# akuendig/cuda-matrix-inversion

Measured on AMD Instinct MI355X. Metric: matrix inversions/s, higher is better.
Workload: dtype f64; 1 GPU; gj64: 100000 x 64x64 fp64 Gauss-Jordan, SPD inputs (natural-order pivots verified inside the MFMA sweep; a rejected matrix is redone with partial pivoting), BASELINE configs[2]; n=64, total_batch=100000, batch_per_gpu=100000, algorithm=gj, kernel=matinv_gj_tile_f64<4, true, true>, input=SPD: R + R^T + n I

## Files before the change

cuda-matrix-inversion_amd/_lib.py:

```python
from __future__ import annotations

import ctypes
import os
import subprocess

_HERE = os.path.dirname(os.path.abspath(__file__))
LIB_PATH = os.environ.get("MATINV_LIB", os.path.join(_HERE, "libmatinv_hip.so"))

OK, ERR_ARG, ERR_UNSUPPORTED, ERR_HIP, ERR_NO_DEVICE = 0, -1, -2, -3, -4
F64, F32 = 0, 1
ALGO_GAUSS_JORDAN, ALGO_CHOLESKY = 0, 1
KERNEL_AUTO, KERNEL_LDS, KERNEL_ROWLANE, KERNEL_TILE, KERNEL_ROW, KERNEL_GLOBAL, KERNEL_BLOCKED, KERNEL_TILEP = 0, 1, 2, 3, 4, 5, 6, 7

REFERENCE_GPU_NAMES = [
    "inverse_gauss_batched_gpu", "inverse_lu_cuda_batched_gpu", "inverse_cholesky_stride_batched_gpu",
    "inverse_cholesky_batched_gpu", "inverse_cholesky_mm_batched_gpu", "inverse_cholesky_mm2_batched_gpu",
]
REFERENCE_DEVICE_NAMES = [
    "inverse_gauss_batched_device", "inverse_lu_cuda_batched_device", "inverse_cholesky_stride_batched_device",
    "decompose_cholesky_stride_batched_device", "inverse_upper_stride_batched_device",
    "multiply_upper_stride_batched_device", "inverse_cholesky_batched_device", "decompose_cholesky_batched_device",
    "inverse_cholesky_mm_batched_device", "decompose_cholesky_mm_batched_device",
    "inverse_cholesky_mm2_batched_device",
]
NATIVE_NAMES = [
    "matinv_inverse_batched", "matinv_inverse_batched_ex", "matinv_select_kernel", "matinv_kernel_name",
    "matinv_mean_batched", "matinv_variance_batched", "matinv_inverse_batched_host", "matinv_mean_batched_host",
    "matinv_variance_batched_host", "matinv_last_error",
    "matinv_abi_version", "matinv_release_cache", "matinv_stream_retire", "matinv_batched_malloc", "matinv_batched_free", "matinv_memcpy_2d",
    "matinv_device_synchronize", "matinv_tile_stats", "matinv_queue_create", "matinv_queue_submit", "matinv_queue_submit_chunks", "matinv_queue_pending",
    "matinv_queue_bins", "matinv_queue_flush", "matinv_queue_destroy", "matinv_queue_last_error", "matinv_queue_stream",
    "matinv_set_gj_policy", "matinv_device_count", "matinv_shard_range", "matinv_inverse_batched_host_multi", "matinv_comm_unique_id",
    "matinv_comm_init_rank", "matinv_comm_destroy", "matinv_allgather_shards", "matinv_allgather_local", "matinv_allgather_local_after", "matinv_debug_rejects",
    "matinv_solve_batched", "matinv_solve_batched_ex", "matinv_solve_kernel_name", "matinv_solve_batched_host",
    "matinv_logdet_batched", "matinv_logdet_batched_ex", "matinv_logdet_kernel_name", "matinv_logdet_batched_host",
    "matinv_logml_batched", "matinv_logml_batched_host", "matinv_gp_kernel_name", "matinv_logml_kernel_name",
    "matinv_loo_batched", "matinv_loo_kernel_name", "matinv_loo_batched_host",
    "matinv_logml_grad_batched", "matinv_logml_grad_kernel_name", "matinv_logml_grad_batched_host",
]
GJ_NATURAL_FIRST, GJ_PIVOT, GJ_ADAPTIVE = 0, 1, 2


def build(force: bool = False) -> str:
    if force:
        subprocess.run(["make", "-C", _HERE, "-s", "clean"], check=True)
    subprocess.run(["make", "-C", _HERE, "-s", "-j4"], check=True)
    return LIB_PATH


class MatinvError(RuntimeError):
    def __init__(self, code: int, msg: str):
        super().__init__(f"libmatinv_hip error {code}: {msg}")
        self.code = code
# ... 65 lines not shown
        f.restype = ci
        f.argtypes = [ci, ci, vp, vp, vp, vp, vp, sz, vp]
    L.matinv_inverse_batched_host_multi.restype = ci
    L.matinv_inverse_batched_host_multi.argtypes = [ci, ci, ci, vp, vp, sz, vp, ci]
    L.matinv_set_gj_policy.restype = ci
    L.matinv_set_gj_policy.argtypes = [ci]
    L.matinv_device_count.restype = ci
    L.matinv_shard_range.restype = ci
    L.matinv_shard_range.argtypes = [sz, ci, ci, ci, vp, vp]
    L.matinv_comm_unique_id.restype = ci
    L.matinv_comm_unique_id.argtypes = [vp]
    L.matinv_comm_init_rank.restype = ci
    L.matinv_comm_init_rank.argtypes = [vp, ci, vp, ci]
    L.matinv_comm_destroy.restype = ci
    L.matinv_comm_destroy.argtypes = [vp]
    L.matinv_allgather_shards.restype = ci
    L.matinv_allgather_shards.argtypes = [vp, ci, vp, vp, sz, vp]
    L.matinv_allgather_local.restype = ci
    L.matinv_allgather_local.argtypes = [ci, vp, ci, vp, vp, sz]
    L.matinv_allgather_local_after.restype = ci
    L.matinv_allgather_local_after.argtypes = [ci, vp, ci, vp, vp, sz, vp]
    L.matinv_tile_stats.restype = ci
    L.matinv_tile_stats.argtypes = [vp, vp, vp, vp]
    L.matinv_batched_malloc.restype = ci
    L.matinv_batched_malloc.argtypes = [vp, vp, sz, ci]
    L.matinv_batched_free.restype = ci
    L.matinv_batched_free.argtypes = [vp]
    L.matinv_memcpy_2d.restype = ci
    L.matinv_memcpy_2d.argtypes = [vp, sz, vp, sz, sz, sz, ci]
    L.matinv_device_synchronize.restype = ci
    L.matinv_queue_create.restype = ci
    L.matinv_queue_create.argtypes = [vp, ci, vp, ci]
    L.matinv_queue_submit.restype = ci
    L.matinv_queue_submit.argtypes = [vp, ci, vp, vp, vp, vp, vp, sz, vp]
    L.matinv_queue_submit_chunks.restype = ci
    L.matinv_queue_submit_chunks.argtypes = [vp, sz, vp, vp, vp, vp, vp, vp, vp, vp]
    L.matinv_queue_pending.restype = ci
    L.matinv_queue_pending.argtypes = [vp, vp, vp]
    L.matinv_queue_bins.restype = ci
    L.matinv_queue_bins.argtypes = [vp, vp, ci]
    L.matinv_queue_flush.restype = ci
    L.matinv_queue_flush.argtypes = [vp, vp, vp, vp]
    L.matinv_queue_stream.restype = vp
    L.matinv_queue_stream.argtypes = [vp]
    L.matinv_queue_destroy.restype = ci
    L.matinv_queue_destroy.argtypes = [vp]
# ... 20 lines not shown
```

cuda-matrix-inversion_amd/api.py:

```python
from __future__ import annotations

import ctypes

import numpy as np

from . import _lib
from ._lib import (GJ_ADAPTIVE, GJ_NATURAL_FIRST, GJ_PIVOT,
                   ALGO_CHOLESKY, ALGO_GAUSS_JORDAN, F32, F64, KERNEL_AUTO, KERNEL_BLOCKED, KERNEL_GLOBAL, KERNEL_LDS,
                   KERNEL_ROW, KERNEL_ROWLANE, KERNEL_TILE, KERNEL_TILEP, MatinvError)


def _np_dtype_code(dtype) -> int:
    dtype = np.dtype(dtype)
    if dtype == np.float64:
        return F64
    if dtype == np.float32:
        return F32
    raise TypeError(f"only float32/float64 batches are supported, got {dtype}")


def _torch_dtype_code(t) -> int:
    import torch
    if t.dtype == torch.float64:
        return F64
# ... 404 lines not shown
    return _lib.lib().matinv_logdet_kernel_name(algo, code, n, kernel).decode()


def gp_kernel_name(dtype, n: int, variance: bool = False) -> str:
    code = dtype if isinstance(dtype, int) else _np_dtype_code(dtype)
    return _lib.lib().matinv_gp_kernel_name(code, n, 1 if variance else 0).decode()


def logml_kernel_name(dtype, n: int) -> str:
    code = dtype if isinstance(dtype, int) else _np_dtype_code(dtype)
    return _lib.lib().matinv_logml_kernel_name(code, n).decode()


mean_batched = calcluateMean
variance_batched = calcluateVariance


def tile_stats() -> dict:
    v = [ctypes.c_ulonglong(0) for _ in range(4)]
    _lib.check(_lib.lib().matinv_tile_stats(*[ctypes.byref(x) for x in v]))
    return dict(zip(("natural_launches", "pivot_launches", "last_rejected", "last_batch"), (int(x.value) for x in v)))


def select_kernel(algo: int, dtype, n: int) -> int:
    code = dtype if isinstance(dtype, int) else _np_dtype_code(dtype)
    k = _lib.lib().matinv_select_kernel(algo, code, n)
    if k < 0:
        _lib.check(k)
    return k


def kernel_name(algo: int, dtype, n: int, kernel: int = KERNEL_AUTO) -> str:
    code = dtype if isinstance(dtype, int) else _np_dtype_code(dtype)
    return _lib.lib().matinv_kernel_name(algo, code, n, kernel).decode()
```

cuda-matrix-inversion_amd/csrc/abi.hip:

```cpp
#include <errno.h>
#include <stdarg.h>
#include <stdio.h>
#include <stdlib.h>
#include <string.h>
#include <time.h>

#include <algorithm>
#include <string>
#include <thread>
#include <vector>

#include "../../include/matinv.h"
#include "common.hpp"

using namespace matinv;

namespace {
thread_local char g_err[512] = "";
}

namespace matinv {
int fail(int code, const char *fmt, ...)
{
    va_list ap;
// ... 1016 lines not shown
    return MATINV_OK;
}

int matinv_memcpy_2d(void *dst, size_t dpitch, const void *src, size_t spitch, size_t width, size_t height, int toDevice)
{
    if (width == 0 || height == 0) return MATINV_OK;
    if (!dst || !src || dpitch < width || spitch < width) return fail(MATINV_ERR_ARG, "matinv_memcpy_2d: bad argument");
    hipError_t e = hipMemcpy2D(dst, dpitch, src, spitch, width, height, toDevice ? hipMemcpyHostToDevice : hipMemcpyDeviceToHost);
    if (e != hipSuccess) return fail_hip(e, "hipMemcpy2D");
    return MATINV_OK;
}

int matinv_tile_stats(unsigned long long *natural_launches, unsigned long long *pivot_launches, unsigned long long *last_rejected,
                      unsigned long long *last_batch)
{
    const TileStats s = tile_stats();
    if (natural_launches) *natural_launches = s.natural_launches;
    if (pivot_launches) *pivot_launches = s.pivot_launches;
    if (last_rejected) *last_rejected = s.last_rejected;
    if (last_batch) *last_batch = s.last_batch;
    return MATINV_OK;
}

int matinv_device_synchronize(void)
{
    hipError_t e = hipDeviceSynchronize();
    if (e != hipSuccess) return fail_hip(e, "hipDeviceSynchronize");
    return MATINV_OK;
}

int matinv_inverse_batched_ex(int algo, int dtype, int n, const void *dA, size_t strideA, void *dAinv,
                              size_t strideInv, size_t batch, int *dInfo, void *stream, int kernel)
{
    if (dtype == MATINV_F64)
        return inverse_strided<double>(algo, n, dA, strideA, dAinv, strideInv, batch, dInfo, stream, kernel);
    if (dtype == MATINV_F32)
        return inverse_strided<float>(algo, n, dA, strideA, dAinv, strideInv, batch, dInfo, stream, kernel);
    return fail(MATINV_ERR_ARG, "unknown dtype %d", dtype);
}

int matinv_inverse_batched(int algo, int dtype, int n, const void *dA, size_t strideA, void *dAinv, size_t strideInv,
                           size_t batch, int *dInfo, void *stream)
{
    return matinv_inverse_batched_ex(algo, dtype, n, dA, strideA, dAinv, strideInv, batch, dInfo, stream,
                                     MATINV_KERNEL_AUTO);
}
// ... 277 lines not shown
```

cuda-matrix-inversion_amd/csrc/common.hpp:

```cpp
#pragma once
#include <hip/hip_runtime.h>
#include <stddef.h>
#include <stdint.h>

#include <type_traits>

#include "../../include/matinv.h"

namespace matinv {

typedef unsigned long long hint_t;

int fail(int code, const char *fmt, ...) __attribute__((format(printf, 2, 3)));
int fail_hip(hipError_t e, const char *what);

hipError_t scratch_alloc(void **p, size_t bytes, hipStream_t stream);
hipError_t scratch_free(void *p, hipStream_t stream);
void scratch_retire_stream(hipStream_t stream);
void blocked_gp_release_graphs();
void scratch_release_device();

template <class Body>
hipError_t with_scratch_ints(size_t count, size_t zeroed, hipStream_t stream, Body &&body)
{
// ... 140 lines not shown

template <class T>
hipError_t launch_gj_tile(int n, BatchRef<const T> A, BatchRef<T> X, size_t batch, int *info, hipStream_t stream);
template <class T>
bool tile_family_supports(int n);
bool tile4_supports(int n);
bool tile4_wide_supports(bool f64, int n);
template <class T>
hipError_t launch_gj_tile4(int n, BatchRef<const T> A, BatchRef<T> X, size_t batch, int *info, hipStream_t stream);
template <class T>
hipError_t launch_spd_tile4(int n, BatchRef<const T> A, BatchRef<T> X, size_t batch, int *info, hipStream_t stream);
const char *name_tile4(bool f64, bool spd, int n);
template <class T>
hipError_t launch_spd_tile(int n, BatchRef<const T> A, BatchRef<T> X, size_t batch, int *info, hipStream_t stream);
template <class T>
bool spd_tile_supports(int n);
const char *name_spd_tile(bool f64, int n);

bool tilep_supports(int n);
template <class T>
hipError_t launch_gj_tilep(int n, BatchRef<const T> A, BatchRef<T> X, size_t batch, int *info, hipStream_t stream);
template <class T>
hipError_t launch_gj_tilep_worklist(int n, BatchRef<const T> A, BatchRef<T> X, size_t batch, const int *in_count, const int *in_list,
                                    int *bad_count, int *bad_list, int *info, hipStream_t stream, hint_t *hint_out, bool expect_many = false);
const char *name_gj_tilep(bool f64, int n);
template <class T>
hipError_t launch_gj_tilep4(int n, BatchRef<const T> A, BatchRef<T> X, size_t batch, int *info, hipStream_t stream);
template <class T>
hipError_t launch_gj_tilep4_worklist(int n, BatchRef<const T> A, BatchRef<T> X, size_t batch, const int *in_count, const int *in_list,
                                     int *bad_count, int *bad_list, int *info, hipStream_t stream, hint_t *hint_out, bool expect_many = false);
const char *name_gj_tilep4(bool f64, int n);
template <class T>
hipError_t launch_gj_tileq(int n, BatchRef<const T> A, BatchRef<T> X, size_t batch, int *info, hipStream_t stream, const int *in_count,
                           const int *in_list, hint_t *hint_out, int *bad_count, int *bad_list);
const char *name_gj_tileq(bool f64, int n);
bool tileq_supports(bool f64, int n);
struct TileStats {
    unsigned long long natural_launches, pivot_launches, last_rejected, last_batch;
};
TileStats tile_stats();
bool tile_policy_use_pivot(bool f64, int nt);
hint_t *tile_policy_record(bool f64, int nt, size_t batch);
int gj_policy();
int set_gj_policy(int policy);

const char *name_gj_rowlane(bool f64, int n);
const char *name_gj_tile(bool f64, int n);
template <class T>
hipError_t launch_gp_lds_worklist(int n, const T *As, const T *Bs, const T *Cs, const T *Ds, const T *Es, T *out,
                                  const int *work_count, const int *work_list, int *info, hipStream_t stream);
bool gp_tile_supports(bool f64, int n);
template <class T>
hipError_t launch_gp_tile(int n, const T *As, const T *Bs, const T *Cs, const T *Ds, const T *Es, T *out, size_t batch,
                          int *info, hipStream_t stream);
const char *name_gp_tile(bool f64, int n);
hipError_t debug_note_rejects(const int *work_count, hipStream_t stream);
long long debug_rejects(bool reset);
bool gp_spd_tile_supports(bool f64, int n);
const char *name_gp_spd_tile(bool f64, int n);
int spd_onewave_max(bool f64);
hipError_t enqueue_spd_tile_wide_f32(int n, BatchRef<const float> A, BatchRef<float> X, unsigned grid, unsigned b, int *info, int *ws,
                                     hipStream_t stream);
hipError_t enqueue_spd_tile_wide_f64(int n, BatchRef<const double> A, BatchRef<double> X, unsigned grid, unsigned b, int *info, int *ws,
                                     hipStream_t stream);
// ... 71 lines not shown
```

cuda-matrix-inversion_amd/csrc/tile_impl.hpp:

```cpp
#pragma once
#include <stdio.h>
#include <stdlib.h>
#include <string.h>
#include <atomic>

#include "tile_common.hpp"
#include "tile_screen.hpp"

#ifndef MATINV_TILE_GATED_PANEL
#define MATINV_TILE_GATED_PANEL 1
#endif

#ifndef MATINV_TILE_SYM_SWEEP
#define MATINV_TILE_SYM_SWEEP 1
#endif

namespace matinv {


#define MATINV_PREP_ROW(MOV, b, a) MOV " %" #b ", %" #a "\n\t" MOV " %" #a ", 0\n\t"
#define MATINV_PREP_ZERO(MOV, a) MOV " %" #a ", 0\n\t"
#define MATINV_PREP_TAIL(MOV, save, eye) MOV " %0, %" #eye "\n\ts_nop 1\n\ts_mov_b64 exec, %" #save
#define MATINV_PREP_SAVE(save, mask) "s_and_saveexec_b64 %" #save ", %" #mask "\n\t"
template <int NT, class T>
__device__ __forceinline__ void prep_operands(typename TileGeo<T>::vec4 (&acc)[NT][NT], T (&bop)[NT], int kb, T eye)
{
    static_assert(NT >= 1 && NT <= 4, "prep_operands: one asm text per tile count");
    const int tK = kb >> 2, rK = kb & 3;
    const unsigned long long pmask = sizeof(T) == 8 ? 0x000F000F000F000FULL << (4 * rK) : 0x1111111111111111ULL << rK;
    unsigned long long save;
    auto J = [&](int i) { return (tK + i) % NT; };
    auto R = [&](int i) { return (rK + i) & 3; };
#define ROW(i) acc[tK][J(i)][rK]
#define COL(i, r) acc[J(i)][tK][R(r)]
    if constexpr (sizeof(T) == 8) {
#define MV "v_mov_b64_e32"
        if constexpr (NT == 1)
// ... 387 lines not shown
            if (info && l == 0) info[mat] = 0;                                                                              \
        } else if (l == 0) {                                                                                                \
            const int slot = atomicAdd(work_count, 1);                                                                      \
            work_list[slot] = (int)mat;                                                                                     \
        }
        if constexpr (SYM) {
            auto leave = [&]() {
                MATINV_GJ_TILE_LEAVE
            };
            if (!sym) {
                leave();
            } else {
                int qs = q, cs = c;
                asm volatile("" : "+v"(qs), "+v"(cs));
                wave_lds_sync();
                sym_tile_sweep<NT, MATINV_TILE_GATED_PANEL != 0, T>(acc, panel, qs, cs, bad);
                wave_lds_sync();
                if (bad == 0) sym_tile_finish<NT>(panel, acc, qs, cs);
                leave();
            }
        } else {
            MATINV_GJ_TILE_LEAVE
        }
#undef MATINV_GJ_TILE_LEAVE
        if (LOOKAHEAD) wave_lds_sync();
    }
}


template <int NT, bool FULL, bool LOOKAHEAD, bool EARLY = false>
__global__ __launch_bounds__(64, 2) void matinv_gj_tile_f64(BatchRef<const double> Ain,
                                                                                 BatchRef<double> Xout, int *info,
                                                                                 int n_rt, unsigned batch,
                                                                                 int *work_count, int *work_list, const int *in_count,
                                                                                 const int *in_list)
{
    constexpr bool SYM = MATINV_TILE_SYM_SWEEP && NT == 4 && FULL && LOOKAHEAD;
    __shared__ __attribute__((aligned(16))) double panel[SYM && 16 * NT * 4 < 16 * TILE_TSTRIDE ? 16 * TILE_TSTRIDE : 16 * NT * 4];
    gj_tile_body<double, NT, FULL, LOOKAHEAD, EARLY>(Ain, Xout, info, n_rt, batch, work_count, work_list, panel, in_count, in_list);
}

template <int NT, bool FULL, bool LOOKAHEAD, bool EARLY = false>
__global__ __launch_bounds__(64, FULL ? 4 : 3) void matinv_gj_tile_f32(BatchRef<const float> Ain, BatchRef<float> Xout, int *info,
                                                           int n_rt, unsigned batch, int *work_count, int *work_list, const int *in_count,
                                                           const int *in_list)
{
    __shared__ __attribute__((aligned(16))) float panel[16 * NT * 4];
    gj_tile_body<float, NT, FULL, LOOKAHEAD, EARLY>(Ain, Xout, info, n_rt, batch, work_count, work_list, panel, in_count, in_list);
}

template <class T>
struct SpdGp {
    const T *a, *c, *d, *e;
    T *out;
};

template <class T, int NT, bool FULL, bool GP = false>
__device__ __forceinline__ void spd_tile_body(BatchRef<const T> Ain, BatchRef<T> Xout, int *info, int n_rt, unsigned batch,
                                              int *work_count, int *work_list, T *panel, SpdGp<T> gp = SpdGp<T>())
{
    typedef TileGeo<T> G;
    typedef typename G::vec4 vec4;
// ... 199 lines not shown
template <int NT>
__global__ __launch_bounds__(64, NT >= 7 ? 1 : 2) void matinv_gp_spd_tile_f64(const double *As, const double *Bs, const double *Cs, const double *Ds,
                                                               const double *Es, double *out, int *info, int n_rt, unsigned batch,
                                                               int *work_count, int *work_list)
{
    __shared__ __attribute__((aligned(16))) double panel[(16 * NT * 4 > 16 * 17) ? 16 * NT * 4 : 16 * 17];
    BatchRef<const double> A{Bs, (size_t)n_rt * n_rt, nullptr};
    BatchRef<double> X{nullptr, 0, nullptr};
    spd_tile_body<double, NT, false, true>(A, X, info, n_rt, batch, work_count, work_list, panel, SpdGp<double>{As, Cs, Ds, Es, out});
}
template <int NT>
__global__ __launch_bounds__(64, NT >= 9 ? MATINV_SPD_WIDE_OCC : 2) void matinv_gp_spd_tile_f32(const float *As, const float *Bs, const float *Cs, const float *Ds,
                                                               const float *Es, float *out, int *info, int n_rt, unsigned batch,
                                                               int *work_count, int *work_list)
{
    __shared__ __attribute__((aligned(16))) float panel[(16 * NT * 4 > 16 * 17) ? 16 * NT * 4 : 16 * 17];
    BatchRef<const float> A{Bs, (size_t)n_rt * n_rt, nullptr};
    BatchRef<float> X{nullptr, 0, nullptr};
    spd_tile_body<float, NT, false, true>(A, X, info, n_rt, batch, work_count, work_list, panel, SpdGp<float>{As, Cs, Ds, Es, out});
}


bool tile_policy_use_screen(bool f64, int nt);
template <class T>
hipError_t launch_gj_tile_natural(int n, BatchRef<const T> A, BatchRef<T> X, size_t batch, int *info, hipStream_t stream)
{
    constexpr bool F64 = sizeof(T) == 8;
    const TileShape s = tile_shape(n);
    const bool rowlane2 = rowlane2_supports(n);
    const bool screen = !rowlane2 && tile_policy_use_screen(F64, s.nt);
    return with_scratch_ints((screen ? 3 : 2) * batch + 4, 4, stream, [&](int *ws) {
        int *const rej_count = ws, *const sing_count = ws + 1, *const acc_count = ws + 2;
        int *const rej_list = ws + 4, *const sing_list = ws + 4 + batch, *const acc_list = ws + 4 + 2 * batch;
        hipError_t e;
        if (rowlane2) {
            e = enqueue_gj_rowlane2<T>(n, A, X, batch, info, stream, rej_count, rej_list);
        } else {
            const unsigned grid = tile_grid(batch, F64 ? 8u : 16u), b = (unsigned)batch;
            const unsigned sgrid = tile_grid(batch, 16u, 1u);
            with_tile<1, 4>(s, [&](auto NT, auto FULL) {
                constexpr bool EARLY = NT >= 3;
                if constexpr (F64) {
                    if (!screen) {
                        hipLaunchKernelGGL((matinv_gj_tile_f64<NT, FULL, true>), dim3(grid), dim3(64), 0, stream, A, X, info, n, b, rej_count,
                                           rej_list, nullptr, nullptr);
                        return;
                    }
                    hipLaunchKernelGGL((matinv_gj_tile_screen_f64<NT, FULL>), dim3(sgrid), dim3(64), 0, stream, A, n, b, rej_count, rej_list,
                                       acc_count, acc_list);
                    hipLaunchKernelGGL((matinv_gj_tile_f64<NT, FULL, true, EARLY>), dim3(grid), dim3(64), 0, stream, A, X, info, n, b, rej_count,
                                       rej_list, acc_count, acc_list);
                } else {
                    if (!screen) {
                        hipLaunchKernelGGL((matinv_gj_tile_f32<NT, FULL, true>), dim3(grid), dim3(64), 0, stream, A, X, info, n, b, rej_count,
                                           rej_list, nullptr, nullptr);
                        return;
                    }
// ... 54 lines not shown
```

cuda-matrix-inversion_amd/csrc/tile_kernels.hip:

```cpp
#include "tile_impl.hpp"

namespace matinv {


unsigned tile_grid_rounds()
{
    static const unsigned rounds = []() {
        const char *s = getenv("MATINV_TILE_GRID_MULT");
        const int v = s && *s ? atoi(s) : 64;
        return (unsigned)(v < 1 ? 1 : v);
    }();
    return rounds;
}

namespace {
constexpr int kMaxDevices = 16, kSlotsPerDevice = 64;
struct HintSlot {
    std::atomic<unsigned long long> pair;
    std::atomic<unsigned> launches_in_pivot_mode;
};
HintSlot *hint_slots()
{
    static HintSlot *slots = []() -> HintSlot * {
        void *p = nullptr;
// ... 57 lines not shown
hint_t *tile_policy_record(bool f64, int nt, size_t batch)
{
    (void)batch;
    if (gj_policy() == MATINV_GJ_PIVOT) return nullptr;
    HintSlot *h = hint_slots();
    if (!h) return nullptr;
    static_assert(sizeof(std::atomic<unsigned long long>) == sizeof(hint_t), "the device stores into the atomic's storage");
    return reinterpret_cast<hint_t *>(&h[slot_index(f64, nt)].pair);
}

bool tile_policy_use_screen(bool f64, int nt)
{
    static const int forced = []() {
        const char *s = getenv("MATINV_TILE_SCREEN");
        return !s || !*s ? -1 : (*s == '0' ? 0 : 1);
    }();
    if (forced >= 0) return forced == 1;
    if (gj_policy() != MATINV_GJ_NATURAL_FIRST) return false;
    HintSlot *h = hint_slots();
    if (!h) return false;
    const unsigned long long pr = h[slot_index(f64, nt)].pair.load(std::memory_order_relaxed);
    const unsigned long long batch = pr >> 32, rejected = pr & 0xffffffffull;
    return batch > 0 && 4ull * rejected >= batch;
}

TileStats tile_stats()
{
    HintSlot *h = hint_slots();
    TileStats t{g_natural_launches.load(), g_pivot_launches.load(), 0, 0};
    if (h) {
        const unsigned long long pr = h[g_last_slot.load()].pair.load(std::memory_order_relaxed);
        t.last_rejected = pr & 0xffffffffull;
        t.last_batch = pr >> 32;
    }
    return t;
}

template <class T>
bool tile_family_supports(int n) { return n >= 1 && n <= (sizeof(T) == 8 ? 192 : 256); }
template <class T>
bool spd_tile_supports(int n) { return n >= 1 && n <= (sizeof(T) == 8 ? 192 : 256); }
template bool tile_family_supports<double>(int);
template bool tile_family_supports<float>(int);
template bool spd_tile_supports<double>(int);
template bool spd_tile_supports<float>(int);

// ... 57 lines not shown
```

cuda-matrix-inversion_amd/csrc/tilep_f32_kernels.hip:

```cpp
#include "tilep_impl.hpp"

namespace matinv {

template hipError_t launch_gj_tilep<float>(int, BatchRef<const float>, BatchRef<float>, size_t, int *, hipStream_t);
template hipError_t launch_gj_tilep_worklist<float>(int, BatchRef<const float>, BatchRef<float>, size_t, const int *, const int *, int *,
                                                    int *, int *, hipStream_t, hint_t *, bool);

}
```

cuda-matrix-inversion_amd/csrc/tilep_impl.hpp:

```cpp
#pragma once
#include <cstdio>
#include <cstdlib>
#include <cstring>

#include "tile_common.hpp"
#include "wave_util.hpp"
#include "gather_tree.inc"

namespace matinv {

template <class T>
struct Vec4Of;
template <>
struct Vec4Of<double> {
    typedef v4d type;
};
template <>
struct Vec4Of<float> {
    typedef v4f type;
};

template <class T, int NT, int TI>
__device__ __forceinline__ void gather_zero_tile_row(typename TileGeo<T>::vec4 (&acc)[NT][NT], unsigned addr, int pos,
                                                    unsigned long long mask)
// ... 81 lines not shown
    lane_rows_swap<WIDE>(alo, blo);
    lane_rows_swap<WIDE>(ahi, bhi);
    a = __longlong_as_double((long long)(((unsigned long long)ahi << 32) | alo));
    b = __longlong_as_double((long long)(((unsigned long long)bhi << 32) | blo));
}

template <class T, int NT, int TI>
__device__ __forceinline__ void gather_row_tree(typename TileGeo<T>::vec4 (&acc)[NT][NT], unsigned addr, int pos, unsigned long long mask)
{
    if constexpr (NT == 1) gather_tree_1x1<4 * TI>(acc[TI][0], addr, pos, mask);
    else if constexpr (NT == 2) gather_tree_2x1<4 * TI>(acc[TI][0], acc[TI][1], addr, pos, mask);
    else if constexpr (NT == 3) gather_tree_3x1<4 * TI>(acc[TI][0], acc[TI][1], acc[TI][2], addr, pos, mask);
    else gather_tree_4x1<4 * TI>(acc[TI][0], acc[TI][1], acc[TI][2], acc[TI][3], addr, pos, mask);
}

template <int V>
struct IntC {
    static constexpr int value = V;
};

template <class T, int NT, bool FULL>
__device__ __forceinline__ void gj_tilep_body(BatchRef<const T> Ain, BatchRef<T> Xout, int *info, int n_rt, unsigned batch,
                                              T *lds, unsigned char *tab, const int *in_count, const int *in_list, hint_t *hint_out,
                                              int *bad_count, int *bad_list)
{
    typedef TileGeo<T> G;
    typedef typename G::vec4 vec4;
    constexpr int N = 16 * NT;
    T *const panel = lds;
    T *const bbuf = lds + 256;
    unsigned char *const rowaddr = tab, *const coladdr = tab + 64;
    const int l = threadIdx.x;
    typedef __attribute__((address_space(3))) T *lds_ptr;
    const unsigned bb_lane = (unsigned)(size_t)(lds_ptr)(bbuf + (l & 15));

    const unsigned todo = in_count ? (unsigned)*in_count : batch;
    if (hint_out && blockIdx.x == 0 && threadIdx.x == 0) __hip_atomic_store(hint_out, ((hint_t)batch << 32) | todo, __ATOMIC_RELAXED, __HIP_MEMORY_SCOPE_SYSTEM);
    for (unsigned item = blockIdx.x; item < todo; item += gridDim.x) {
        const unsigned mat = in_list ? (unsigned)in_list[item] : item;
        const T *A = Ain.at_uniform(mat);
        T *X = Xout.at_uniform(mat);
        int n = FULL ? N : n_rt;
        if (!FULL) asm volatile("" : "+s"(n));
        int q = l >> 4, c = l & 15, lr = l;
        const unsigned lane_off = (unsigned)(G::trow(0, l >> 4) * n + (l & 15));
        asm volatile("" : "+v"(q), "+v"(c), "+v"(lr));

        vec4 acc[NT][NT];
#pragma unroll
        for (int ti = 0; ti < NT; ++ti)
#pragma unroll
            for (int tj = 0; tj < NT; ++tj)
#pragma unroll
                for (int r = 0; r < 4; ++r) {
                    const int row = 16 * ti + G::trow(r, q), col = 16 * tj + c;
                    const unsigned uoff = (unsigned)((16 * ti + G::trow(r, 0)) * n + 16 * tj);
                    const bool edge = !FULL && (ti == NT - 1 || tj == NT - 1);
                    acc[ti][tj][r] = (!edge || (row < n && col < n)) ? A[uoff + lane_off] : ((row == col) ? (T)1 : (T)0);
                }

// ... 170 lines not shown
            for (int tj = 0; tj < NT; ++tj) ca[tj] = coladdr[16 * tj + c];
#pragma unroll
            for (int ti = 0; ti < NT; ++ti)
#pragma unroll
                for (int r = 0; r < 4; ++r) {
                    const unsigned ra = rowaddr[16 * ti + G::trow(r, q)];
#pragma unroll
                    for (int tj = 0; tj < NT; ++tj) {
                        if (FULL || (ra < (unsigned)n && ca[tj] < (unsigned)n)) X[ra * (unsigned)n + ca[tj]] = acc[ti][tj][r];
                    }
                }
            if (info && l == 0) info[mat] = 0;
        } else if (l == 0) {
            const int slot = atomicAdd(bad_count, 1);
            bad_list[slot] = (int)mat;
        }
        wave_lds_sync();
    }
}

template <int NT, bool FULL>
__global__ __launch_bounds__(64, 3) void matinv_gj_tilep_f64(BatchRef<const double> Ain, BatchRef<double> Xout, int *info, int n_rt,
                                                            unsigned batch, const int *in_count, const int *in_list, hint_t *hint_out,
                                                            int *bad_count, int *bad_list)
{
    __shared__ __attribute__((aligned(16))) double lds[256 + 4 * 16 * NT];
    __shared__ unsigned char tab[128];
    gj_tilep_body<double, NT, FULL>(Ain, Xout, info, n_rt, batch, lds, tab, in_count, in_list, hint_out, bad_count, bad_list);
}

template <int NT, bool FULL>
__global__ __launch_bounds__(64, 3) void matinv_gj_tilep_f32(BatchRef<const float> Ain, BatchRef<float> Xout, int *info, int n_rt,
                                                            unsigned batch, const int *in_count, const int *in_list, hint_t *hint_out,
                                                            int *bad_count, int *bad_list)
{
    __shared__ __attribute__((aligned(16))) float lds[256 + 4 * 16 * NT];
    __shared__ unsigned char tab[128];
    gj_tilep_body<float, NT, FULL>(Ain, Xout, info, n_rt, batch, lds, tab, in_count, in_list, hint_out, bad_count, bad_list);
}

template <class T>
static hipError_t enqueue_tilep(int n, BatchRef<const T> A, BatchRef<T> X, size_t batch, int *info, hipStream_t stream,
                                const int *in_count, const int *in_list, hint_t *hint_out, int *bad_count, int *bad_list, bool expect_many = false)
{
    const unsigned grid = in_list && !expect_many ? tile_grid(batch, 12u, 1u) : tile_grid(batch, 12u), b = (unsigned)batch;
    with_tile<1, 4>(tile_shape(n), [&](auto NT, auto FULL) {
        if constexpr (sizeof(T) == 8)
            hipLaunchKernelGGL((matinv_gj_tilep_f64<NT, FULL>), dim3(grid), dim3(64), 0, stream, A, X, info, n, b, in_count, in_list, hint_out,
                               bad_count, bad_list);
        else
            hipLaunchKernelGGL((matinv_gj_tilep_f32<NT, FULL>), dim3(grid), dim3(64), 0, stream, A, X, info, n, b, in_count, in_list, hint_out,
                               bad_count, bad_list);
    });
    return hipGetLastError();
}

template <class T>
hipError_t launch_gj_tilep(int n, BatchRef<const T> A, BatchRef<T> X, size_t batch, int *info, hipStream_t stream)
{
    if (n < 1 || n > 64) return hipErrorInvalidValue;
    if (batch == 0) return hipSuccess;
    return with_scratch_ints(batch + 1, 1, stream, [&](int *ws) {
        hipError_t e = enqueue_tilep<T>(n, A, X, batch, info, stream, nullptr, nullptr, nullptr, ws, ws + 1);
        if (e == hipSuccess) e = launch_gj_row_worklist<T>(n, A, X, ws, ws + 1, info, stream);
        return e;
    });
}

template <class T>
hipError_t launch_gj_tilep_worklist(int n, BatchRef<const T> A, BatchRef<T> X, size_t batch, const int *in_count, const int *in_list,
                                    int *bad_count, int *bad_list, int *info, hipStream_t stream, hint_t *hint_out, bool expect_many)
{
    hipError_t e = enqueue_tilep<T>(n, A, X, batch, info, stream, in_count, in_list, hint_out, bad_count, bad_list, expect_many);
    if (e == hipSuccess) e = launch_gj_row_worklist<T>(n, A, X, bad_count, bad_list, info, stream);
    if (e == hipSuccess) e = debug_note_rejects(in_count, stream);
    return e;
}

}
```

cuda-matrix-inversion_amd/csrc/tilep_kernels.hip:

```cpp
#include "tilep_impl.hpp"

namespace matinv {

bool tilep_supports(int n) { return n >= 1 && n <= 128; }

template hipError_t launch_gj_tilep<double>(int, BatchRef<const double>, BatchRef<double>, size_t, int *, hipStream_t);
template hipError_t launch_gj_tilep_worklist<double>(int, BatchRef<const double>, BatchRef<double>, size_t, const int *, const int *, int *,
                                                     int *, int *, hipStream_t, hint_t *, bool);

const char *name_gj_tilep(bool f64, int n)
{
    if (n > 64) return name_gj_tilep4(f64, n);
    const TileShape s = tile_shape(n);
    static thread_local char buf[48];
    snprintf(buf, sizeof buf, "matinv_gj_tilep_%s<%d, %s>", f64 ? "f64" : "f32", s.nt, s.full ? "true" : "false");
    return buf;
}

}
```

include/matinv.h:

```cpp
#ifndef MATINV_H_INCLUDED
#define MATINV_H_INCLUDED

#include <stddef.h>

#ifdef __cplusplus
extern "C" {
#endif

typedef enum {
    MATINV_OK = 0,
    MATINV_ERR_ARG = -1,
    MATINV_ERR_UNSUPPORTED = -2,
    MATINV_ERR_HIP = -3,
    MATINV_ERR_NO_DEVICE = -4
} matinv_status;

typedef enum {
    MATINV_F64 = 0,
    MATINV_F32 = 1
} matinv_dtype;

typedef enum {
    MATINV_ALGO_GAUSS_JORDAN = 0,
    MATINV_ALGO_CHOLESKY = 1
// ... 72 lines not shown
                                      int nshards);
int matinv_device_count(void);
int matinv_shard_range(size_t batch, int nshards, int n, int g, size_t *lo, size_t *hi);

int matinv_comm_unique_id(void *id128);
int matinv_comm_init_rank(void **comm, int nranks, const void *id128, int rank);
int matinv_comm_destroy(void *comm);
int matinv_allgather_shards(void *comm, int dtype, const void *dSend, void *dRecv, size_t count, void *stream);
int matinv_allgather_local(int ndev, const int *devices, int dtype, const void *const *dSend, void *const *dRecv, size_t count);
int matinv_allgather_local_after(int ndev, const int *devices, int dtype, const void *const *dSend, void *const *dRecv, size_t count,
                                 void *const *producer_streams);

int matinv_mean_batched_host(int dtype, int n, const void *hAs, const void *hBs, const void *hCs, const void *hDs,
                             void *hMeans, size_t batch, int *info);
int matinv_variance_batched_host(int dtype, int n, const void *hAs, const void *hBs, const void *hCs, const void *hEs,
                                 void *hVars, size_t batch, int *info);

int matinv_batched_malloc(void **devArrayPtr, size_t *pitch, size_t arraySize, int batchSize);
int matinv_batched_free(void **devArrayPtr);
int matinv_memcpy_2d(void *dst, size_t dpitch, const void *src, size_t spitch, size_t width, size_t height, int toDevice);
int matinv_device_synchronize(void);
int matinv_tile_stats(unsigned long long *natural_launches, unsigned long long *pivot_launches, unsigned long long *last_rejected,
                      unsigned long long *last_batch);

typedef struct matinv_queue matinv_queue;
int matinv_queue_create(matinv_queue **q, int dtype, const int *bins, int nbins);
int matinv_queue_submit(matinv_queue *q, int n, const void *dAs, const void *dBs, const void *dCs, const void *dDs,
                        const void *dEs, size_t count, size_t *first_ticket);
int matinv_queue_submit_chunks(matinv_queue *q, size_t chunks, const int *n, const void *const *dAs, const void *const *dBs,
                               const void *const *dCs, const void *const *dDs, const void *const *dEs, const size_t *count,
                               size_t *first_tickets);
int matinv_queue_pending(const matinv_queue *q, size_t *items, size_t *per_bin);
int matinv_queue_bins(const matinv_queue *q, int *bins, int cap);
int matinv_queue_flush(matinv_queue *q, void *dMeans, void *dVariances, void *stream);
void *matinv_queue_stream(matinv_queue *q);
int matinv_queue_destroy(matinv_queue *q);
const char *matinv_queue_last_error(const matinv_queue *q);

const char *matinv_last_error(void);
int matinv_abi_version(void);

int matinv_release_cache(void);
int matinv_stream_retire(void *stream);

long long matinv_debug_rejects(int reset);

// ... 5 lines not shown
```

Baseline: 76.77 million inversions/s.

## Add symmetric-only front kernel for 64x64 fp64 Gauss-Jordan with fallback worklist

Adds a dedicated kernel for 64x64 fp64 that loads each matrix into registers, checks symmetry through LDS transposes, and runs only the symmetric sweep path. Matrices that are not symmetric are appended to a worklist, which the general tile kernel then processes. An adaptive host policy drops the front kernel (probing every 32nd launch) when at least a quarter of matrices turn out non-symmetric. The front kernel is meant to use a smaller, specialised code path and higher occupancy (12 workgroups per CU), at the cost of an extra symmetry check and one more launch.

```diff
diff --git a/cuda-matrix-inversion_amd/_lib.py b/cuda-matrix-inversion_amd/_lib.py
--- a/cuda-matrix-inversion_amd/_lib.py
+++ b/cuda-matrix-inversion_amd/_lib.py
@@ -28,7 +28,7 @@
     "matinv_mean_batched", "matinv_variance_batched", "matinv_inverse_batched_host", "matinv_mean_batched_host",
     "matinv_variance_batched_host", "matinv_last_error",
     "matinv_abi_version", "matinv_release_cache", "matinv_stream_retire", "matinv_batched_malloc", "matinv_batched_free", "matinv_memcpy_2d",
-    "matinv_device_synchronize", "matinv_tile_stats", "matinv_queue_create", "matinv_queue_submit", "matinv_queue_submit_chunks", "matinv_queue_pending",
+    "matinv_device_synchronize", "matinv_tile_stats", "matinv_sym_front_stats", "matinv_queue_create", "matinv_queue_submit", "matinv_queue_submit_chunks", "matinv_queue_pending",
     "matinv_queue_bins", "matinv_queue_flush", "matinv_queue_destroy", "matinv_queue_last_error", "matinv_queue_stream",
     "matinv_set_gj_policy", "matinv_device_count", "matinv_shard_range", "matinv_inverse_batched_host_multi", "matinv_comm_unique_id",
     "matinv_comm_init_rank", "matinv_comm_destroy", "matinv_allgather_shards", "matinv_allgather_local", "matinv_allgather_local_after", "matinv_debug_rejects",
@@ -140,6 +140,9 @@
     L.matinv_allgather_local_after.argtypes = [ci, vp, ci, vp, vp, sz, vp]
     L.matinv_tile_stats.restype = ci
     L.matinv_tile_stats.argtypes = [vp, vp, vp, vp]
+    if hasattr(L, "matinv_sym_front_stats"):
+        L.matinv_sym_front_stats.restype = ci
+        L.matinv_sym_front_stats.argtypes = [vp, vp, vp, vp]
     L.matinv_batched_malloc.restype = ci
     L.matinv_batched_malloc.argtypes = [vp, vp, sz, ci]
     L.matinv_batched_free.restype = ci
diff --git a/cuda-matrix-inversion_amd/api.py b/cuda-matrix-inversion_amd/api.py
--- a/cuda-matrix-inversion_amd/api.py
+++ b/cuda-matrix-inversion_amd/api.py
@@ -450,6 +450,12 @@
     return dict(zip(("natural_launches", "pivot_launches", "last_rejected", "last_batch"), (int(x.value) for x in v)))
 
 
+def sym_front_stats() -> dict:
+    v = [ctypes.c_ulonglong(0) for _ in range(4)]
+    _lib.check(_lib.lib().matinv_sym_front_stats(*[ctypes.byref(x) for x in v]))
+    return dict(zip(("front_launches", "direct_launches", "last_not_symmetric", "last_batch"), (int(x.value) for x in v)))
+
+
 def select_kernel(algo: int, dtype, n: int) -> int:
     code = dtype if isinstance(dtype, int) else _np_dtype_code(dtype)
     k = _lib.lib().matinv_select_kernel(algo, code, n)
diff --git a/cuda-matrix-inversion_amd/csrc/abi.hip b/cuda-matrix-inversion_amd/csrc/abi.hip
--- a/cuda-matrix-inversion_amd/csrc/abi.hip
+++ b/cuda-matrix-inversion_amd/csrc/abi.hip
@@ -1062,6 +1062,17 @@
     return MATINV_OK;
 }
 
+int matinv_sym_front_stats(unsigned long long *front_launches, unsigned long long *direct_launches, unsigned long long *last_not_symmetric,
+                           unsigned long long *last_batch)
+{
+    const SymFrontStats s = sym_front_stats();
+    if (front_launches) *front_launches = s.front_launches;
+    if (direct_launches) *direct_launches = s.direct_launches;
+    if (last_not_symmetric) *last_not_symmetric = s.last_not_symmetric;
+    if (last_batch) *last_batch = s.last_batch;
+    return MATINV_OK;
+}
+
 int matinv_device_synchronize(void)
 {
     hipError_t e = hipDeviceSynchronize();
diff --git a/cuda-matrix-inversion_amd/csrc/common.hpp b/cuda-matrix-inversion_amd/csrc/common.hpp
--- a/cuda-matrix-inversion_amd/csrc/common.hpp
+++ b/cuda-matrix-inversion_amd/csrc/common.hpp
@@ -186,7 +186,8 @@
 hipError_t launch_gj_tilep(int n, BatchRef<const T> A, BatchRef<T> X, size_t batch, int *info, hipStream_t stream);
 template <class T>
 hipError_t launch_gj_tilep_worklist(int n, BatchRef<const T> A, BatchRef<T> X, size_t batch, const int *in_count, const int *in_list,
-                                    int *bad_count, int *bad_list, int *info, hipStream_t stream, hint_t *hint_out, bool expect_many = false);
+                                    int *bad_count, int *bad_list, int *info, hipStream_t stream, hint_t *hint_out, bool expect_many = false,
+                                    const int *aux_count = nullptr, hint_t *aux_out = nullptr);
 const char *name_gj_tilep(bool f64, int n);
 template <class T>
 hipError_t launch_gj_tilep4(int n, BatchRef<const T> A, BatchRef<T> X, size_t batch, int *info, hipStream_t stream);
@@ -204,6 +205,10 @@
 };
 TileStats tile_stats();
 bool tile_policy_use_pivot(bool f64, int nt);
+struct SymFrontStats {
+    unsigned long long front_launches, direct_launches, last_not_symmetric, last_batch;
+};
+SymFrontStats sym_front_stats();
 hint_t *tile_policy_record(bool f64, int nt, size_t batch);
 int gj_policy();
 int set_gj_policy(int policy);
diff --git a/cuda-matrix-inversion_amd/csrc/tile_impl.hpp b/cuda-matrix-inversion_amd/csrc/tile_impl.hpp
--- a/cuda-matrix-inversion_amd/csrc/tile_impl.hpp
+++ b/cuda-matrix-inversion_amd/csrc/tile_impl.hpp
@@ -13,6 +13,10 @@
 
 #ifndef MATINV_TILE_SYM_SWEEP
 #define MATINV_TILE_SYM_SWEEP 1
+#endif
+
+#ifndef MATINV_TILE_SYM_FRONT
+#define MATINV_TILE_SYM_FRONT 1
 #endif
 
 namespace matinv {
@@ -446,10 +450,87 @@
         } else {
             MATINV_GJ_TILE_LEAVE
         }
-#undef MATINV_GJ_TILE_LEAVE
         if (LOOKAHEAD) wave_lds_sync();
     }
 }
+
+
+constexpr int sym_cls_ti(int k) { return k < 6 ? (k < 1 ? 1 : (k < 3 ? 2 : 3)) : k - 6; }
+constexpr int sym_cls_tj(int k) { return k < 6 ? (k < 1 ? 0 : (k < 3 ? k - 1 : k - 3)) : k - 6; }
+
+template <int CB>
+__device__ __forceinline__ bool tile_symmetric_batched(double *tbuf, const v4d (&acc)[4][4], int q, int c)
+{
+    typedef TileGeo<double> G;
+    constexpr int NITEM = 10, TSZ = 16 * TILE_TSTRIDE;
+    unsigned long long asym = 0;
+#pragma unroll
+    for (int g = 0; g < NITEM; g += CB) {
+        wave_lds_sync();
+#pragma unroll
+        for (int k = g; k < g + CB && k < NITEM; ++k)
+#pragma unroll
+            for (int r = 0; r < 4; ++r) tbuf[(k - g) * TSZ + G::trow(r, q) * TILE_TSTRIDE + c] = acc[sym_cls_ti(k)][sym_cls_tj(k)][r];
+        wave_lds_sync();
+#pragma unroll
+        for (int k = g; k < g + CB && k < NITEM; ++k)
+#pragma unroll
+            for (int r = 0; r < 4; ++r)
+                note_differs(asym, tbuf[(k - g) * TSZ + c * TILE_TSTRIDE + G::trow(r, q)], acc[sym_cls_tj(k)][sym_cls_ti(k)][r]);
+    }
+    return asym == 0;
+}
+
+constexpr int TILE_SYM_CLS_BATCH = 5;
+
+__device__ __forceinline__ void gj_tile_sym_body(BatchRef<const double> Ain, BatchRef<double> Xout, int *info, unsigned batch, int *work_count,
+                                                 int *work_list, int *ns_count, int *ns_list, double *panel)
+{
+    typedef double T;
+    typedef TileGeo<T> G;
+    typedef typename G::vec4 vec4;
+    typedef typename G::vec2 vec2;
+    constexpr int NT = 4, N = 16 * NT;
+    constexpr bool FULL = true, PAIRED = true;
+    const int l = threadIdx.x;
+
+    for (unsigned mat = blockIdx.x; mat < batch; mat += gridDim.x) {
+        const T *A = Ain.at_uniform(mat);
+        T *X = Xout.at_uniform(mat);
+        constexpr int n = N;
+        constexpr unsigned lane_off = 0;
+        int q = l >> 4, c = l & 15;
+        asm volatile("" : "+v"(q), "+v"(c));
+        vec4 acc[NT][NT];
+        {
+            const unsigned lane_off2 = (unsigned)(2 * G::trow(0, l >> 4) * N + 2 * (l & 15));
+#pragma unroll
+            for (int ti = 0; ti < NT; ++ti)
+#pragma unroll
+                for (int u = 0; u < NT / 2; ++u)
+#pragma unroll
+                    for (int r = 0; r < 4; ++r) {
+                        const unsigned uoff = (unsigned)((32 * (ti >> 1) + 2 * G::trow(r, 0) + (ti & 1)) * N + 32 * u);
+                        const vec2 v = __builtin_nontemporal_load(reinterpret_cast<const vec2 *>(A + uoff + lane_off2));
+                        acc[ti][2 * u][r] = v[0];
+                        acc[ti][2 * u + 1][r] = v[1];
+                    }
+        }
+        unsigned long long bad = 0;
+        if (tile_symmetric_batched<TILE_SYM_CLS_BATCH>(panel, acc, q, c)) {
+            wave_lds_sync();
+            sym_tile_sweep<NT, MATINV_TILE_GATED_PANEL != 0, T>(acc, panel, q, c, bad);
+            wave_lds_sync();
+            if (bad == 0) sym_tile_finish<NT>(panel, acc, q, c);
+            MATINV_GJ_TILE_LEAVE
+        } else if (l == 0) {
+            const int slot = atomicAdd(ns_count, 1);
+            ns_list[slot] = (int)mat;
+        }
+        wave_lds_sync();
+    }
+}
+#undef MATINV_GJ_TILE_LEAVE
 
 
 template <int NT, bool FULL, bool LOOKAHEAD, bool EARLY = false>
@@ -462,6 +543,17 @@
     constexpr bool SYM = MATINV_TILE_SYM_SWEEP && NT == 4 && FULL && LOOKAHEAD;
     __shared__ __attribute__((aligned(16))) double panel[SYM && 16 * NT * 4 < 16 * TILE_TSTRIDE ? 16 * TILE_TSTRIDE : 16 * NT * 4];
     gj_tile_body<double, NT, FULL, LOOKAHEAD, EARLY>(Ain, Xout, info, n_rt, batch, work_count, work_list, panel, in_count, in_list);
+}
+
+template <int NT, bool FULL, bool LOOKAHEAD, bool EARLY, bool SYMONLY>
+__global__ __launch_bounds__(64, 3) void matinv_gj_tile_f64(BatchRef<const double> Ain, BatchRef<double> Xout, int *info, int n_rt,
+                                                            unsigned batch, int *work_count, int *work_list, int *ns_count, int *ns_list)
+{
+    static_assert(NT == 4 && FULL && LOOKAHEAD && !EARLY && SYMONLY, "the symmetric-only form exists at 64 x 64 only");
+    (void)n_rt;
+    __shared__ __attribute__((aligned(16))) double panel[TILE_SYM_CLS_BATCH * 16 * TILE_TSTRIDE];
+    static_assert(sizeof(panel) >= sizeof(double) * 16 * NT * 4 && 12 * sizeof(panel) <= 160 * 1024, "panel + transpose buffers, 12 workgroups per CU");
+    gj_tile_sym_body(Ain, Xout, info, batch, work_count, work_list, ns_count, ns_list, panel);
 }
 
 template <int NT, bool FULL, bool LOOKAHEAD, bool EARLY = false>
@@ -707,6 +799,8 @@
 
 
 bool tile_policy_use_screen(bool f64, int nt);
+bool tile_policy_use_sym_front(int nt);
+hint_t *tile_policy_record_sym_front(int nt);
 template <class T>
 hipError_t launch_gj_tile_natural(int n, BatchRef<const T> A, BatchRef<T> X, size_t batch, int *info, hipStream_t stream)
 {
@@ -714,10 +808,25 @@
     const TileShape s = tile_shape(n);
     const bool rowlane2 = rowlane2_supports(n);
     const bool screen = !rowlane2 && tile_policy_use_screen(F64, s.nt);
-    return with_scratch_ints((screen ? 3 : 2) * batch + 4, 4, stream, [&](int *ws) {
-        int *const rej_count = ws, *const sing_count = ws + 1, *const acc_count = ws + 2;
-        int *const rej_list = ws + 4, *const sing_list = ws + 4 + batch, *const acc_list = ws + 4 + 2 * batch;
+    const bool front = MATINV_TILE_SYM_FRONT && MATINV_TILE_SYM_SWEEP && F64 && n == 64 && !screen && tile_policy_use_sym_front(s.nt);
+    return with_scratch_ints((screen || front ? 3 : 2) * batch + 4, 4, stream, [&](int *ws) {
+        int *const rej_count = ws, *const sing_count = ws + 1, *const acc_count = ws + 2, *const ns_count = ws + 3;
+        int *const rej_list = ws + 4, *const sing_list = ws + 4 + batch, *const acc_list = ws + 4 + 2 * batch, *const ns_list = acc_list;
         hipError_t e;
+        if constexpr (F64) {
+            if (front) {
+                const unsigned b = (unsigned)batch;
+                hipLaunchKernelGGL((matinv_gj_tile_f64<4, true, true, false, true>), dim3(tile_grid(batch, 12u)), dim3(64), 0, stream, A, X, info,
+                                   n, b, rej_count, rej_list, ns_count, ns_list);
+                hipLaunchKernelGGL((matinv_gj_tile_f64<4, true, true>), dim3(tile_grid(batch, 8u, 1u)), dim3(64), 0, stream, A, X, info, n, b,
+                                   rej_count, rej_list, ns_count, ns_list);
+                e = hipGetLastError();
+                if (e == hipSuccess)
+                    e = launch_gj_tilep_worklist<T>(n, A, X, batch, rej_count, rej_list, sing_count, sing_list, info, stream,
+                                                    tile_policy_record(F64, s.nt, batch), false, ns_count, tile_policy_record_sym_front(s.nt));
+                return e;
+            }
+        }
         if (rowlane2) {
             e = enqueue_gj_rowlane2<T>(n, A, X, batch, info, stream, rej_count, rej_list);
         } else {
diff --git a/cuda-matrix-inversion_amd/csrc/tile_kernels.hip b/cuda-matrix-inversion_amd/csrc/tile_kernels.hip
--- a/cuda-matrix-inversion_amd/csrc/tile_kernels.hip
+++ b/cuda-matrix-inversion_amd/csrc/tile_kernels.hip
@@ -103,6 +103,62 @@
     const unsigned long long pr = h[slot_index(f64, nt)].pair.load(std::memory_order_relaxed);
     const unsigned long long batch = pr >> 32, rejected = pr & 0xffffffffull;
     return batch > 0 && 4ull * rejected >= batch;
+}
+
+namespace {
+struct FrontSlot {
+    std::atomic<unsigned long long> pair;
+    std::atomic<unsigned> launches_in_direct_mode;
+};
+FrontSlot *front_slots()
+{
+    static FrontSlot *slots = []() -> FrontSlot * {
+        void *p = nullptr;
+        if (hipHostMalloc(&p, sizeof(FrontSlot) * kMaxDevices * kSlotsPerDevice, hipHostMallocPortable) != hipSuccess) return nullptr;
+        memset(p, 0, sizeof(FrontSlot) * kMaxDevices * kSlotsPerDevice);
+        return static_cast<FrontSlot *>(p);
+    }();
+    return slots;
+}
+std::atomic<unsigned long long> g_front_launches{0}, g_direct_launches{0};
+std::atomic<int> g_last_front_slot{0};
+}
+
+bool tile_policy_use_sym_front(int nt)
+{
+    FrontSlot *h = front_slots();
+    bool front = h != nullptr;
+    if (h) {
+        const int idx = slot_index(true, nt);
+        g_last_front_slot.store(idx, std::memory_order_relaxed);
+        const unsigned long long pr = h[idx].pair.load(std::memory_order_relaxed);
+        const unsigned long long batch = pr >> 32, notsym = pr & 0xffffffffull;
+        if (batch > 0 && 4ull * notsym >= batch)
+            front = ((h[idx].launches_in_direct_mode.fetch_add(1, std::memory_order_relaxed) + 1) % 32u) == 0;
+        else
+            h[idx].launches_in_direct_mode.store(0, std::memory_order_relaxed);
+    }
+    (front ? g_front_launches : g_direct_launches).fetch_add(1, std::memory_order_relaxed);
+    return front;
+}
+
+hint_t *tile_policy_record_sym_front(int nt)
+{
+    FrontSlot *h = front_slots();
+    static_assert(sizeof(std::atomic<unsigned long long>) == sizeof(hint_t), "the device stores into the atomic's storage");
+    return h ? reinterpret_cast<hint_t *>(&h[slot_index(true, nt)].pair) : nullptr;
+}
+
+SymFrontStats sym_front_stats()
+{
+    FrontSlot *h = front_slots();
+    SymFrontStats t{g_front_launches.load(), g_direct_launches.load(), 0, 0};
+    if (h) {
+        const unsigned long long pr = h[g_last_front_slot.load()].pair.load(std::memory_order_relaxed);
+        t.last_not_symmetric = pr & 0xffffffffull;
+        t.last_batch = pr >> 32;
+    }
+    return t;
 }
 
 TileStats tile_stats()
diff --git a/cuda-matrix-inversion_amd/csrc/tilep_f32_kernels.hip b/cuda-matrix-inversion_amd/csrc/tilep_f32_kernels.hip
--- a/cuda-matrix-inversion_amd/csrc/tilep_f32_kernels.hip
+++ b/cuda-matrix-inversion_amd/csrc/tilep_f32_kernels.hip
@@ -4,6 +4,6 @@
 
 template hipError_t launch_gj_tilep<float>(int, BatchRef<const float>, BatchRef<float>, size_t, int *, hipStream_t);
 template hipError_t launch_gj_tilep_worklist<float>(int, BatchRef<const float>, BatchRef<float>, size_t, const int *, const int *, int *,
-                                                    int *, int *, hipStream_t, hint_t *, bool);
+                                                    int *, int *, hipStream_t, hint_t *, bool, const int *, hint_t *);
 
 }
diff --git a/cuda-matrix-inversion_amd/csrc/tilep_impl.hpp b/cuda-matrix-inversion_amd/csrc/tilep_impl.hpp
--- a/cuda-matrix-inversion_amd/csrc/tilep_impl.hpp
+++ b/cuda-matrix-inversion_amd/csrc/tilep_impl.hpp
@@ -127,7 +127,7 @@
 template <class T, int NT, bool FULL>
 __device__ __forceinline__ void gj_tilep_body(BatchRef<const T> Ain, BatchRef<T> Xout, int *info, int n_rt, unsigned batch,
                                               T *lds, unsigned char *tab, const int *in_count, const int *in_list, hint_t *hint_out,
-                                              int *bad_count, int *bad_list)
+                                              int *bad_count, int *bad_list, const int *aux_count, hint_t *aux_out)
 {
     typedef TileGeo<T> G;
     typedef typename G::vec4 vec4;
@@ -141,6 +141,8 @@
 
     const unsigned todo = in_count ? (unsigned)*in_count : batch;
     if (hint_out && blockIdx.x == 0 && threadIdx.x == 0) __hip_atomic_store(hint_out, ((hint_t)batch << 32) | todo, __ATOMIC_RELAXED, __HIP_MEMORY_SCOPE_SYSTEM);
+    if (aux_out && blockIdx.x == 0 && threadIdx.x == 0)
+        __hip_atomic_store(aux_out, ((hint_t)batch << 32) | (unsigned)*aux_count, __ATOMIC_RELAXED, __HIP_MEMORY_SCOPE_SYSTEM);
     for (unsigned item = blockIdx.x; item < todo; item += gridDim.x) {
         const unsigned mat = in_list ? (unsigned)in_list[item] : item;
         const T *A = Ain.at_uniform(mat);
@@ -357,35 +359,36 @@
 template <int NT, bool FULL>
 __global__ __launch_bounds__(64, 3) void matinv_gj_tilep_f64(BatchRef<const double> Ain, BatchRef<double> Xout, int *info, int n_rt,
                                                             unsigned batch, const int *in_count, const int *in_list, hint_t *hint_out,
-                                                            int *bad_count, int *bad_list)
+                                                            int *bad_count, int *bad_list, const int *aux_count, hint_t *aux_out)
 {
     __shared__ __attribute__((aligned(16))) double lds[256 + 4 * 16 * NT];
     __shared__ unsigned char tab[128];
-    gj_tilep_body<double, NT, FULL>(Ain, Xout, info, n_rt, batch, lds, tab, in_count, in_list, hint_out, bad_count, bad_list);
+    gj_tilep_body<double, NT, FULL>(Ain, Xout, info, n_rt, batch, lds, tab, in_count, in_list, hint_out, bad_count, bad_list, aux_count, aux_out);
 }
 
 template <int NT, bool FULL>
 __global__ __launch_bounds__(64, 3) void matinv_gj_tilep_f32(BatchRef<const float> Ain, BatchRef<float> Xout, int *info, int n_rt,
                                                             unsigned batch, const int *in_count, const int *in_list, hint_t *hint_out,
-                                                            int *bad_count, int *bad_list)
+                                                            int *bad_count, int *bad_list, const int *aux_count, hint_t *aux_out)
 {
     __shared__ __attribute__((aligned(16))) float lds[256 + 4 * 16 * NT];
     __shared__ unsigned char tab[128];
-    gj_tilep_body<float, NT, FULL>(Ain, Xout, info, n_rt, batch, lds, tab, in_count, in_list, hint_out, bad_count, bad_list);
+    gj_tilep_body<float, NT, FULL>(Ain, Xout, info, n_rt, batch, lds, tab, in_count, in_list, hint_out, bad_count, bad_list, aux_count, aux_out);
 }
 
 template <class T>
 static hipError_t enqueue_tilep(int n, BatchRef<const T> A, BatchRef<T> X, size_t batch, int *info, hipStream_t stream,
-                                const int *in_count, const int *in_list, hint_t *hint_out, int *bad_count, int *bad_list, bool expect_many = false)
+                                const int *in_count, const int *in_list, hint_t *hint_out, int *bad_count, int *bad_list, bool expect_many = false,
+                                const int *aux_count = nullptr, hint_t *aux_out = nullptr)
 {
     const unsigned grid = in_list && !expect_many ? tile_grid(batch, 12u, 1u) : tile_grid(batch, 12u), b = (unsigned)batch;
     with_tile<1, 4>(tile_shape(n), [&](auto NT, auto FULL) {
         if constexpr (sizeof(T) == 8)
             hipLaunchKernelGGL((matinv_gj_tilep_f64<NT, FULL>), dim3(grid), dim3(64), 0, stream, A, X, info, n, b, in_count, in_list, hint_out,
-                               bad_count, bad_list);
+                               bad_count, bad_list, aux_count, aux_out);
         else
             hipLaunchKernelGGL((matinv_gj_tilep_f32<NT, FULL>), dim3(grid), dim3(64), 0, stream, A, X, info, n, b, in_count, in_list, hint_out,
-                               bad_count, bad_list);
+                               bad_count, bad_list, aux_count, aux_out);
     });
     return hipGetLastError();
 }
@@ -404,9 +407,10 @@
 
 template <class T>
 hipError_t launch_gj_tilep_worklist(int n, BatchRef<const T> A, BatchRef<T> X, size_t batch, const int *in_count, const int *in_list,
-                                    int *bad_count, int *bad_list, int *info, hipStream_t stream, hint_t *hint_out, bool expect_many)
-{
-    hipError_t e = enqueue_tilep<T>(n, A, X, batch, info, stream, in_count, in_list, hint_out, bad_count, bad_list, expect_many);
+                                    int *bad_count, int *bad_list, int *info, hipStream_t stream, hint_t *hint_out, bool expect_many,
+                                    const int *aux_count, hint_t *aux_out)
+{
+    hipError_t e = enqueue_tilep<T>(n, A, X, batch, info, stream, in_count, in_list, hint_out, bad_count, bad_list, expect_many, aux_count, aux_out);
     if (e == hipSuccess) e = launch_gj_row_worklist<T>(n, A, X, bad_count, bad_list, info, stream);
     if (e == hipSuccess) e = debug_note_rejects(in_count, stream);
     return e;
diff --git a/cuda-matrix-inversion_amd/csrc/tilep_kernels.hip b/cuda-matrix-inversion_amd/csrc/tilep_kernels.hip
--- a/cuda-matrix-inversion_amd/csrc/tilep_kernels.hip
+++ b/cuda-matrix-inversion_amd/csrc/tilep_kernels.hip
@@ -6,7 +6,7 @@
 
 template hipError_t launch_gj_tilep<double>(int, BatchRef<const double>, BatchRef<double>, size_t, int *, hipStream_t);
 template hipError_t launch_gj_tilep_worklist<double>(int, BatchRef<const double>, BatchRef<double>, size_t, const int *, const int *, int *,
-                                                     int *, int *, hipStream_t, hint_t *, bool);
+                                                     int *, int *, hipStream_t, hint_t *, bool, const int *, hint_t *);
 
 const char *name_gj_tilep(bool f64, int n)
 {
diff --git a/include/matinv.h b/include/matinv.h
--- a/include/matinv.h
+++ b/include/matinv.h
@@ -118,6 +118,8 @@
 int matinv_device_synchronize(void);
 int matinv_tile_stats(unsigned long long *natural_launches, unsigned long long *pivot_launches, unsigned long long *last_rejected,
                       unsigned long long *last_batch);
+int matinv_sym_front_stats(unsigned long long *front_launches, unsigned long long *direct_launches, unsigned long long *last_not_symmetric,
+                           unsigned long long *last_batch);
 
 typedef struct matinv_queue matinv_queue;
 int matinv_queue_create(matinv_queue **q, int dtype, const int *bins, int nbins);
```

New measurement: 80.18 million inversions/s, median of 6. 4.4% higher.
